# theAdamColton/dct-autoencoder

Measured on AMD Instinct MI355X. Metric: Mpix/s encode (DCT+PatchNorm+LFQ), patch14 512²; 1/2/4/8 GPU, %HBM roofline, higher is better.
Workload: dtype f32; 1 GPU; fused encode of 512x512 RGB images, patch14, max_patch 32x32, S=3072, LFQ 14 codebooks x 2^14, beta=0; global_batch=1024, parallelism=dp1 (image shards, no collective)

## Files before the change

dct-autoencoder_amd/csrc/dctae_fft2.hip:

```cpp
#include "dctae_device.h"
#include "dctae_fft_common.h"
#include "dctae_launch.h"
#include "dctae_spec512.h"

namespace dctae {

__device__ __forceinline__ constexpr int pad16(int m) { return m + (m >> 4); }

template <int N>
struct RowsLds {
  static constexpr int M = N / 2;
  static constexpr int MP = pad16(M - 1) + 2;
  float2 z[4][3][MP];
};

template <int N, int R1, int R2, typename Px>
__device__ __forceinline__ void rows2_item(const ImgDesc& d, int y_first, const Px* __restrict__ rgb,
                                           float* __restrict__ T, RowsLds<N>& L, const float2* post_s,
                                           const float2* tw_s, const ColorMats& cm) {
  constexpr int M = N / 2;
  constexpr int MP = RowsLds<N>::MP;
  constexpr int B1 = M / R1, B2 = M / R2;
  constexpr int PX = (N + 63) / 64;
  constexpr int KI = (M + 63) / 64;
// ... 458 lines not shown
        if (jl < KS && sk.codes) sk.codes[tok * KS + jl] = (uint16_t)code;
        if (sk.raw && jl < KS) {
#pragma unroll
          for (int p2 = 0; p2 < KS; ++p2) sk.raw[tok * KS * KS + jl * KS + p2] = row[p2];
        }
      }
    }
  } else {
    for (int h = g16; h < d.qh; h += 16) {
      float vals[KS];
      const float* row = zs + (KS * h + jl) * KSP;
#pragma unroll
      for (int p2 = 0; p2 < KS; ++p2) vals[p2] = row[p2];
      const int f = (h * d.qw + strip) * ep.C + c;
      token_epilogue_p<KS>(ep, c, h, strip, jl, vals, d.tok_off + f, sk);
    }
  }
}

template <bool THR, int IPB, bool PF>
__device__ __forceinline__ void cols7_block(int b, const ImgDesc* __restrict__ imgs, const int* __restrict__ list,
                                            int n_list, int n_items, int qw, const float* __restrict__ ws,
                                            const float2* __restrict__ tw, const float2* __restrict__ post,
                                            const EncParams& ep, const TokenSinks& sk, Cols7Lds& L, float4* post4,
                                            float2* tw_s, float* sbias) {
  constexpr int M = 256;
  const int per_x = (n_items + 7) / 8;
  const int slot = b >> 3;
  const int t = (b & 7) * per_x + slot % per_x, g = slot / per_x;
  const int k0 = g * IPB;
  if (t >= n_items || k0 >= n_list) return;
  const int c = t / qw, strip = t - c * qw;
  const float4* p4 = reinterpret_cast<const float4*>(post);
  for (int i = threadIdx.x; i < M + 1; i += 256) post4[i] = p4[i];
  for (int i = threadIdx.x; i < M; i += 256) tw_s[i] = tw[i];
  float2 thr_r[2][7];
  cols_thresholds<THR>(imgs[list[k0]], c, strip, ep, thr_r, sbias);
  float va[16], vb[16];
  {
    const ImgDesc d0 = imgs[list[k0]];
    cols7_load(d0, c, strip, ws + d0.ws_t, va, vb);
  }
  __syncthreads();
#pragma unroll
  for (int u = 0; u < IPB; ++u) {
    const int k = k0 + u;
    if (k < n_list) {
      const ImgDesc dk = imgs[list[k]];
      if (u > 0 && !PF) cols7_load(dk, c, strip, ws + dk.ws_t, va, vb);
#pragma unroll
      for (int r = 0; r < 16; ++r) asm volatile("" : "+v"(va[r]), "+v"(vb[r]));
      float na[16], nb[16];
      if (PF && u + 1 < IPB) {
        const ImgDesc dn = imgs[list[min(k + 1, n_list - 1)]];
        cols7_load(dn, c, strip, ws + dn.ws_t, na, nb);
      }
      cols7_compute<THR>(dk, c, strip, L, va, vb, post4, tw_s, sbias, thr_r, ep, sk);
      __syncthreads();
      if (PF && u + 1 < IPB) {
#pragma unroll
        for (int r = 0; r < 16; ++r) {
          va[r] = na[r];
          vb[r] = nb[r];
        }
      }
    }
  }
}

template <bool THR, int IPB, bool PF>
__global__ __launch_bounds__(256) void k_fft_cols7(const ImgDesc* __restrict__ imgs, const int* __restrict__ list,
                                                   int n_list, int n_items, int qw,
                                                   const float* __restrict__ ws, const float2* __restrict__ tw,
                                                   const float2* __restrict__ post, EncParams ep, TokenSinks sk) {
  __shared__ Cols7Lds L;
  __shared__ float4 post4[257];
  __shared__ float2 tw_s[256];
  __shared__ float sbias[32];
  cols7_block<THR, IPB, PF>(blockIdx.x, imgs, list, n_list, n_items, qw, ws, tw, post, ep, sk, L, post4, tw_s, sbias);
}

constexpr int kC5bIpb = 3;
constexpr int kC5bNormIpb = 3;
template <bool THR, int IPB, bool NORM = false>
__global__ __launch_bounds__(256) void k_cols512b(const ImgDesc* __restrict__ imgs, const int* __restrict__ list,
                                                  int n_list, const float* __restrict__ ws,
                                                  const float2* __restrict__ tw, const float2* __restrict__ post,
                                                  EncParams ep, TokenSinks sk) {
  constexpr int M = 256, per_x = 12;
  __shared__ Cols512bLds L;
  const int b = blockIdx.x;
  const int slot = b >> 3;
  const int t = (b & 7) * per_x + slot % per_x, k0 = (slot / per_x) * IPB;
  if (k0 >= n_list) return;
  const int c = t >> 5, strip = t & 31;
  const int tid = threadIdx.x;
  L.tw2[tid >> 4][tid & 15] = tw[(tid >> 4) * (tid & 15)];
  const float4* p4 = reinterpret_cast<const float4*>(post);
  {
    const float4 ab = p4[tid];
    L.pc[tid] = make_float4(ab.x + ab.z, ab.x - ab.z, ab.y + ab.w, ab.y - ab.w);
  }
  const float4 abM = p4[M];
  const float4 pcM = make_float4(abM.x + abM.z, abM.x - abM.z, abM.y + abM.w, abM.y - abM.w);
  float2 thr_r[2][7];
  cols_thresholds<THR>(imgs[list[k0]], c, strip, ep, thr_r, nullptr);
  float sb[2] = {0.0f, 0.0f};
  if (THR || NORM) {
    const int g16 = tid >> 4;
    sb[0] = __fdiv_rn(-(float)(g16 + strip), ep.ci[c]);
    sb[1] = __fdiv_rn(-(float)(g16 + 16 + strip), ep.ci[c]);
  }
  float2 tn[NORM ? 2 : 1][14];
  if constexpr (NORM) cols_norm_tables(c, strip, ep, tn);
  float4 qa[8];
  cols512b_load(c, strip, ws + imgs[list[k0]].ws_t, qa);
  __syncthreads();
#pragma unroll
  for (int u = 0; u < IPB; ++u) {
    const int k = k0 + u;
    if (k < n_list) {
      const ImgDesc dk = imgs[list[k]];
      t_opaque(qa);
      float4 qn[8];
      if (u + 1 < IPB) cols512b_load(c, strip, ws + imgs[list[min(k + 1, n_list - 1)]].ws_t, qn);
      float4 qf[8];
      t_decode(qa, qf);
      cols512b_compute<THR, NORM>(dk, c, strip, L, qf, pcM, sb, thr_r, ep, sk, tn);
      __syncthreads();
      if (u + 1 < IPB) {
#pragma unroll
        for (int r = 0; r < 8; ++r) qa[r] = qn[r];
      }
    }
  }
}

struct Cols512wLds {
  union {
    cf xch[28][kXchStridePk];
    float X[2][449 * 14];
  } u;
  uint32_t rmax[2][32][14];
  float2 tw2[16][16];
  float4 pc[256];
};

__device__ __forceinline__ void cols512w_load(int c, int kx, const float* __restrict__ T, float4 (&q)[8]) {
  t_load_column(c, kx, opaque_tid() & 15, T, q);
}

__device__ __forceinline__ void cols512w_transform(Cols512wLds& L, const float4 (&qa)[8], float4 pcM) {
#pragma clang fp contract(fast)
  constexpr int N = 512, M = 256, KS = 14;
  const int tid = opaque_tid();
  const int G = tid >> 4, j = tid & 15;
  const int sg = G >= KS ? 1 : 0, col = G - KS * sg;
  const int s = sigma16(j);
  const bool self0 = (j == 0), self8 = (j == 15);
  cf v[16];
#pragma unroll
  for (int bb = 0; bb < 8; ++bb) {
    v[bb] = (cf){qa[bb].x, qa[bb].y};
    v[15 - bb] = (cf){mirror16(qa[bb].z), mirror16(qa[bb].w)};
  }
  fft256_group(v, L.u.xch[G], j, s, L.tw2);
  __syncthreads();
  float* xs = L.u.X[sg];
  float* xa = xs + s * KS + col;
  float* xb = xs + (N - s) * KS + col;
  float4 cn0 = L.pc[s], cn1 = L.pc[s + 16];
#pragma unroll
  for (int i = 0; i < 16; i += 2) {
    const float4 c0 = cn0, c1 = cn1;
    if (i + 2 < 16) {
      cn0 = L.pc[s + 16 * (i + 2)];
      cn1 = L.pc[s + 16 * (i + 3)];
    }
    cf x0, x1;
    makhoul_step2(v, i, self0, self8, c0, c1, x0, x1);
    xa[224 * i] = x0.x;
    xa[224 * (i + 1)] = x1.x;
    if (i >= 4) xb[-224 * i] = x0.y;
    if (i + 1 >= 4) xb[-224 * (i + 1)] = x1.y;
  }
  if (self0) xs[M * KS + col] = (pcM.x + pcM.y) * v[0].x + (pcM.w - pcM.z) * v[0].y;
}

__device__ __forceinline__ void cols512w_epilogue(Cols512wLds& L, const ImgDesc& dk, int c, int sp,
                                                  const float2 (&thr_r)[2][7], const EncParams& ep,
                                                  const TokenSinks& sk) {
  constexpr int KS = 14;
  const int tid = opaque_tid();
  const int eh = tid / KS, ejl = tid - KS * eh;
  const f2v* row0 = reinterpret_cast<const f2v*>(L.u.X[0]) + (KS * eh + ejl) * (KS / 2);
  const f2v* row1 = reinterpret_cast<const f2v*>(L.u.X[1]) + (KS * eh + ejl) * (KS / 2);
  uint32_t code0 = 0, code1 = 0;
  float am0 = 0.0f, am1 = 0.0f;
#pragma unroll
  for (int p = 0; p < KS / 2; ++p) code_bits4(code0, code1, am0, am1, row0[p], row1[p], thr_r[0][p], thr_r[1][p]);
  L.rmax[0][eh][ejl] = __float_as_uint(am0);
  L.rmax[1][eh][ejl] = __float_as_uint(am1);
  if (sk.codes) {
    sk.codes[cols_tok(dk, c, 2 * sp, eh, ep.C) * KS + ejl] = (uint16_t)code0;
    sk.codes[cols_tok(dk, c, 2 * sp + 1, eh, ep.C) * KS + ejl] = (uint16_t)code1;
  }
  if (sk.raw) {
    for (int e = tid; e < 2 * 32 * 49; e += 448) {
      const int r = e / (32 * 49), e2 = e - r * 32 * 49, h = e2 / 49, q = e2 - h * 49;
      reinterpret_cast<float4*>(sk.raw + cols_tok(dk, c, 2 * sp + r, h, ep.C) * (KS * KS))[q] =
          reinterpret_cast<const float4*>(L.u.X[r] + KS * KS * h)[q];
// ... 10 lines not shown
    uint32_t m = 0;
#pragma unroll
    for (int q = 0; q < KS; ++q) m = max(m, L.rmax[r][h][q]);
    const float sb = __fdiv_rn(-(float)(h + 2 * sp + r), ep.ci[c]);
    sk.scores[cols_tok(dk, c, 2 * sp + r, h, ep.C)] = __fadd_rn(__fmul_rn(__uint_as_float(m), ep.mw), sb);
  }
}

template <int IPB>
__global__ __launch_bounds__(448) __attribute__((amdgpu_waves_per_eu(4))) void k_cols512w(
    const ImgDesc* __restrict__ imgs, const int* __restrict__ list, int n_list, const float* __restrict__ ws,
    const float2* __restrict__ tw, const float2* __restrict__ post, EncParams ep, TokenSinks sk) {
  constexpr int M = 256, KS = 14, per_x = 6;
  __shared__ Cols512wLds L;
  const int b = blockIdx.x;
  const int slot = b >> 3;
  const int t = (b & 7) * per_x + slot % per_x, k0 = (slot / per_x) * IPB;
  if (k0 >= n_list) return;
  const int c = t >> 4, sp = t & 15;
  {
    const int tid = threadIdx.x;
    if (tid < 256) {
      L.tw2[tid >> 4][tid & 15] = tw[(tid >> 4) * (tid & 15)];
      const float4 ab = reinterpret_cast<const float4*>(post)[tid];
      L.pc[tid] = make_float4(ab.x + ab.z, ab.x - ab.z, ab.y + ab.w, ab.y - ab.w);
    }
  }
  const float4 abM = reinterpret_cast<const float4*>(post)[M];
  const float4 pcM = make_float4(abM.x + abM.z, abM.x - abM.z, abM.y + abM.w, abM.y - abM.w);
  float2 thr_r[2][7];
  {
    const int tid = opaque_tid();
    const int eh = tid / KS, ejl = tid - KS * eh;
#pragma unroll
    for (int r = 0; r < 2; ++r) {
      const float2* t2 = reinterpret_cast<const float2*>(
          ep.thr + ((((int64_t)c * ep.maxph + eh) * ep.maxpw) + 2 * sp + r) * (KS * KS) + (int64_t)ejl * KS);
#pragma unroll
      for (int p = 0; p < KS / 2; ++p) thr_r[r][p] = t2[p];
    }
  }
  const int kx = [&] {
    const int G = opaque_tid() >> 4, sg = G >= KS ? 1 : 0;
    return KS * (2 * sp + sg) + G - KS * sg;
  }();
  float4 qa[8];
  cols512w_load(c, kx, ws + imgs[list[k0]].ws_t, qa);
  __syncthreads();
#pragma unroll
  for (int u = 0; u < IPB; ++u) {
    const int k = k0 + u;
    if (k >= n_list) break;
    t_opaque(qa);
    float4 qn[8];
    if (u + 1 < IPB) cols512w_load(c, kx, ws + imgs[list[min(k + 1, n_list - 1)]].ws_t, qn);
    if (u > 0) cols512w_scores(L, imgs[list[k - 1]], c, sp, ep, sk);
    float4 qf[8];
    t_decode(qa, qf);
    cols512w_transform(L, qf, pcM);
    __syncthreads();
    cols512w_epilogue(L, imgs[list[k]], c, sp, thr_r, ep, sk);
    __syncthreads();
    if (u + 1 < IPB) {
#pragma unroll
      for (int r = 0; r < 8; ++r) qa[r] = qn[r];
    }
  }
  cols512w_scores(L, imgs[list[min(k0 + IPB, n_list) - 1]], c, sp, ep, sk);
}

void launch_cols512b(const ImgDesc* imgs, const int* list, int n_list, const float* ws, const float2* tw,
                     const float2* post, const EncParams& ep, const TokenSinks& sk, hipStream_t s, bool wide) {
  if (n_list <= 0) return;
  const bool thr = ep.median && ep.thr && !sk.norm && ep.maxph <= 32 && ep.cb_dim == 14 && ep.ncb == 14;
  const bool norm = !thr && sk.norm && ep.median && !sk.raw && ep.maxph == 32 && ep.maxpw == 32 &&
                    (!sk.codes || (ep.cb_dim == 14 && ep.ncb == 14));
  const int ipb = thr ? kC5bIpb : norm ? kC5bNormIpb : 2;
  const int grid = 96 * ((n_list + ipb - 1) / ipb);
  if (thr && wide) {
    hipLaunchKernelGGL((k_cols512w<kC5bIpb>), dim3(48 * ((n_list + kC5bIpb - 1) / kC5bIpb)), dim3(448), 0, s, imgs,
                       list, n_list, ws, tw, post, ep, sk);
    return;
  }
  if (thr)
    hipLaunchKernelGGL((k_cols512b<true, kC5bIpb>), dim3(grid), dim3(256), 0, s, imgs, list, n_list, ws, tw, post, ep,
                       sk);
  else if (norm)
    hipLaunchKernelGGL((k_cols512b<false, kC5bNormIpb, true>), dim3(grid), dim3(256), 0, s, imgs, list, n_list, ws, tw,
                       post, ep, sk);
  else
    hipLaunchKernelGGL((k_cols512b<false, 2>), dim3(grid), dim3(256), 0, s, imgs, list, n_list, ws, tw, post, ep, sk);
}

int cols7_grid(int n_list, int qw, int ipb) {
  const int n_items = 3 * qw, per_x = (n_items + 7) / 8;
  return 8 * per_x * ((n_list + ipb - 1) / ipb);
}

template <int N, int R2, int KS, bool THR>
__global__ __launch_bounds__(256) void k_fft_cols4(const ImgDesc* __restrict__ imgs, const int4* __restrict__ blocks,
                                                   const float* __restrict__ ws, const float2* __restrict__ tw,
                                                   const float2* __restrict__ post, EncParams ep, TokenSinks sk) {
  constexpr int M = N / 2;
  __shared__ ColsLds<N> L;
  __shared__ float2 post_s[2 * (M + 1)];
  __shared__ float2 tw_s[M];
  __shared__ float sbias[32];
  for (int i = threadIdx.x; i < 2 * (M + 1); i += 256) post_s[i] = post[i];
  for (int i = threadIdx.x; i < M; i += 256) tw_s[i] = tw[i];
  const int4 jb = blocks[blockIdx.x];
  const ImgDesc d = imgs[jb.x];
  cols4_item<N, R2, KS, THR>(d, jb.y, jb.z, ws + d.ws_t, L.z, post_s, tw_s, sbias, ep, sk);
}

template <bool THR>
__global__ __launch_bounds__(256) void k_cols224(const ImgDesc* __restrict__ imgs, const int4* __restrict__ blocks,
                                                 int n_items, const float* __restrict__ ws,
                                                 const float2* __restrict__ tw, const float2* __restrict__ post,
                                                 EncParams ep, TokenSinks sk) {
#pragma clang fp contract(fast)
  constexpr int N = 224, M = 112, R1 = 16, R2 = 7, B1 = 7, KS = 14;
  constexpr int KSP = 30;
  static_assert(KSP >= 2 * KS, "28 columns");
  constexpr int ZROWS = 2 * (pad16(M - 1) + 1);
  static_assert(N <= ZROWS, "natural rows fit the complex layout");
  __shared__ float zs[ZROWS * KSP];
  __shared__ float4 pc[M + 1];
  __shared__ float2 tw_s[M];
  __shared__ float sbias[2][16];
  {
    const float4* p4 = reinterpret_cast<const float4*>(post);
    for (int i = threadIdx.x; i < M + 1; i += 256) {
      const float4 ab = p4[i];
      pc[i] = make_float4(ab.x + ab.z, ab.x - ab.z, ab.y + ab.w, ab.y - ab.w);
    }
    for (int i = threadIdx.x; i < M; i += 256) tw_s[i] = tw[i];
  }
  const int n_pairs = (n_items + 1) / 2, per_x = (n_pairs + 7) / 8;
  const int pidx = (int)(blockIdx.x & 7) * per_x + (int)(blockIdx.x >> 3);
  if (pidx >= n_pairs) return;
  const int tid = opaque_tid();
  const int i0 = 2 * pidx;
  const int4 ja = blocks[i0], jb = blocks[i0 + 1 < n_items ? i0 + 1 : i0];
  const ImgDesc da = imgs[ja.x], db = imgs[jb.x];
  const int g16 = tid >> 4, jl = tid & 15, jlc = min(jl, KS - 1);
  if (THR) {
    if (tid < 32) {
      const int u = tid >> 4, h = tid & 15;
      const int c = u ? jb.y : ja.y, strip = u ? jb.z : ja.z;
      sbias[u][h] = __fdiv_rn(-(float)(h + strip), ep.ci[c]);
    }
  }
  if (tid < 224) {
    const int u = tid >= 112 ? 1 : 0, t = tid - 112 * u;
    const int y0 = t / (KS / 2), p = t - y0 * (KS / 2);
    const int c = u ? jb.y : ja.y, strip = u ? jb.z : ja.z;
    const int64_t tbase = u ? db.ws_t : da.ws_t;
    const int H = u ? db.H : da.H, Kw = u ? db.Kw : da.Kw;
    const c4f2* src = reinterpret_cast<const c4f2*>(ws + tbase + ((int64_t)c * H + y0) * Kw + strip * KS) + p;
    const int64_t rstep = (int64_t)8 * Kw;
    c4f2 tv[N / 16];
#pragma unroll
    for (int k = 0; k < N / 16; ++k) tv[k] = src[k * rstep];
    float* dst = zs + y0 * KSP + KS * u + 2 * p;
#pragma unroll
    for (int k = 0; k < N / 16; ++k) {
      dst[16 * KSP * k] = tv[k].x;
// ... 238 lines not shown
```

dct-autoencoder_amd/csrc/dctae_rows512.h:

```cpp
#pragma once
#include "dctae_device.h"
#include "dctae_fft_common.h"
#include "dctae_pixel.h"

namespace dctae {

typedef unsigned v4u __attribute__((ext_vector_type(4)));

#ifndef DCTAE_TLAYOUT
#define DCTAE_TLAYOUT 2
#endif
static_assert(DCTAE_TLAYOUT == 0 || DCTAE_TLAYOUT == 2, "T' layouts: 0 or 2");
__device__ __forceinline__ int t4_index(int band4, int kx) {
#if DCTAE_TLAYOUT == 0
  return band4 * 448 + kx;
#else
  return ((band4 >> 2) * 448 + kx) * 4 + (band4 & 3);
#endif
}
constexpr int kTStAux = 2, kTLdAux = 2;

__device__ __forceinline__ int u4_index(int band4, int kx) { return ((band4 >> 2) * 448 + kx) * 4 + (band4 & 3); }
constexpr int kUStAux = 2;

// ... 34 lines not shown
  asm("v_pk_mul_f32 %0, %1, %2 op_sel_hi:[1,0] neg_hi:[1,0]" : "=v"(t) : "v"(A), "v"(c12));
  asm("v_pk_fma_f32 %0, %1, %2, %3 op_sel:[0,1,0] op_sel_hi:[1,1,1]" : "=v"(t) : "v"(P), "v"(c12), "v"(t));
  asm("v_pk_fma_f32 %0, %1, %2, %3 op_sel:[1,0,0] op_sel_hi:[0,0,1] neg_lo:[1,0,0] neg_hi:[1,0,0]"
      : "=v"(t) : "v"(A), "v"(c34), "v"(t));
  asm("v_pk_fma_f32 %0, %1, %2, %3 op_sel:[1,1,0] op_sel_hi:[0,1,1] neg_hi:[1,0,0]"
      : "=v"(t) : "v"(P), "v"(c34), "v"(t));
  return t;
}

__device__ __forceinline__ int sigma16(int j) { return j < 8 ? j : (j < 15 ? j + 1 : 8); }

__device__ __forceinline__ void fft256_group(cf (&v)[16], cf* xr, int j, int s, const float2 (&tw2)[16][16]) {
#pragma clang fp contract(fast)
  DFTV<16>::run(v);
#pragma unroll
  for (int k1 = 0; k1 < 16; ++k1) xr[16 * k1 + (j ^ (k1 & 14))] = v[k1];
  __builtin_amdgcn_fence(__ATOMIC_RELEASE, "wavefront");
  __builtin_amdgcn_wave_barrier();
  __builtin_amdgcn_fence(__ATOMIC_ACQUIRE, "wavefront");
  {
    const float4* rr = reinterpret_cast<const float4*>(xr + 16 * s);
    const int sw = s >> 1;
#pragma unroll
    for (int q = 0; q < 8; ++q) {
      const float4 a = rr[q ^ sw];
      v[2 * q] = (cf){a.x, a.y};
      v[2 * q + 1] = (cf){a.z, a.w};
    }
  }
  __builtin_amdgcn_fence(__ATOMIC_RELEASE, "wavefront");
  __builtin_amdgcn_wave_barrier();
#pragma unroll
  for (int r = 1; r < 16; ++r) {
    const float2 w = tw2[r][s];
    v[r] = cmul_pk(v[r], (cf){w.x, w.y});
  }
  DFTV<16>::run(v);
}

__device__ __forceinline__ cf makhoul_step(const cf (&v)[16], int i, int s, bool self0, bool self8,
                                           const float4* pc) {
  const cf m = (cf){mirror16(v[15 - i].x), mirror16(v[15 - i].y)};
  const cf own = self0 ? v[(16 - i) & 15] : v[15 - i];
  const cf P = (self0 || self8) ? own : m;
  const float4 cc = pc[s + 16 * i];
  return makhoul_pair(v[i], P, (cf){cc.x, cc.y}, (cf){cc.z, cc.w});
}

__device__ __forceinline__ void makhoul_pair2(cf A0, cf P0, float4 c0, cf A1, cf P1, float4 c1, cf& t0, cf& t1) {
  const cf c12a = (cf){c0.x, c0.y}, c34a = (cf){c0.z, c0.w}, c12b = (cf){c1.x, c1.y}, c34b = (cf){c1.z, c1.w};
  asm("v_pk_mul_f32 %0, %2, %3 op_sel_hi:[1,0] neg_hi:[1,0]\n\t"
      "v_pk_mul_f32 %1, %6, %7 op_sel_hi:[1,0] neg_hi:[1,0]\n\t"
      "v_pk_fma_f32 %0, %4, %3, %0 op_sel:[0,1,0] op_sel_hi:[1,1,1]\n\t"
      "v_pk_fma_f32 %1, %8, %7, %1 op_sel:[0,1,0] op_sel_hi:[1,1,1]\n\t"
      "v_pk_fma_f32 %0, %2, %5, %0 op_sel:[1,0,0] op_sel_hi:[0,0,1] neg_lo:[1,0,0] neg_hi:[1,0,0]\n\t"
      "v_pk_fma_f32 %1, %6, %9, %1 op_sel:[1,0,0] op_sel_hi:[0,0,1] neg_lo:[1,0,0] neg_hi:[1,0,0]\n\t"
      "v_pk_fma_f32 %0, %4, %5, %0 op_sel:[1,1,0] op_sel_hi:[0,1,1] neg_hi:[1,0,0]\n\t"
      "v_pk_fma_f32 %1, %8, %9, %1 op_sel:[1,1,0] op_sel_hi:[0,1,1] neg_hi:[1,0,0]"
      : "=&v"(t0), "=&v"(t1)
      : "v"(A0), "v"(c12a), "v"(P0), "v"(c34a), "v"(A1), "v"(c12b), "v"(P1), "v"(c34b));
}

__device__ __forceinline__ void makhoul_step2(const cf (&v)[16], int i, bool self0, bool self8, float4 c0, float4 c1,
                                              cf& x0, cf& x1) {
  (void)self0;
  (void)self8;
  float p0x, p0y, p1x, p1y, q0x, q0y, q1x, q1y;
  asm("s_mov_b32 vcc_lo, 0x00010001\n\t"
      "s_mov_b32 vcc_hi, 0x00010001\n\t"
      "v_cndmask_b32 %4, %8, %12, vcc\n\t"
      "v_cndmask_b32 %5, %9, %13, vcc\n\t"
      "v_cndmask_b32 %6, %10, %8, vcc\n\t"
      "v_cndmask_b32 %7, %11, %9, vcc\n\t"
      "s_mov_b32 vcc_lo, 0x80018001\n\t"
      "s_mov_b32 vcc_hi, 0x80018001\n\t"
      "v_cndmask_b32_dpp %0, %8, %4, vcc row_mirror row_mask:0xf bank_mask:0xf\n\t"
      "v_cndmask_b32_dpp %1, %9, %5, vcc row_mirror row_mask:0xf bank_mask:0xf\n\t"
      "v_cndmask_b32_dpp %2, %10, %6, vcc row_mirror row_mask:0xf bank_mask:0xf\n\t"
      "v_cndmask_b32_dpp %3, %11, %7, vcc row_mirror row_mask:0xf bank_mask:0xf"
      : "=&v"(p0x), "=&v"(p0y), "=&v"(p1x), "=&v"(p1y), "=&v"(q0x), "=&v"(q0y), "=&v"(q1x), "=&v"(q1y)
      : "v"(v[15 - i].x), "v"(v[15 - i].y), "v"(v[14 - i].x), "v"(v[14 - i].y), "v"(v[(16 - i) & 15].x),
        "v"(v[(16 - i) & 15].y)
      : "vcc");
  makhoul_pair2(v[i], (cf){p0x, p0y}, c0, v[i + 1], (cf){p1x, p1y}, c1, x0, x1);
}

__device__ __forceinline__ void xpose4_rows(float (&r)[4]) {
  const auto a = __builtin_amdgcn_permlane32_swap(__float_as_uint(r[0]), __float_as_uint(r[2]), false, false);
  const auto b = __builtin_amdgcn_permlane32_swap(__float_as_uint(r[1]), __float_as_uint(r[3]), false, false);
  const auto c = __builtin_amdgcn_permlane16_swap(a[0], b[0], false, false);
  const auto d = __builtin_amdgcn_permlane16_swap(a[1], b[1], false, false);
  r[0] = __uint_as_float(c[0]);
  r[1] = __uint_as_float(c[1]);
  r[2] = __uint_as_float(d[0]);
  r[3] = __uint_as_float(d[1]);
}

template <bool band, typename Px>
__device__ __forceinline__ void rows512_item_pk(Rows512XchPk& X, const Rows512Tab& L, const Px* __restrict__ img,
                                                int H, int y0, float* T, uint32_t plane_bytes, const ColorMats& cm) {
#pragma clang fp contract(fast)
  constexpr int N = 512, M = 256, KW = 448;
  const int tid = threadIdx.x;
  const int wv = tid >> 6, g = (tid >> 4) & 3, j = tid & 15;
  const int y = y0 + 4 * wv + g;
  const int yl = min(y, H - 1);
  const int64_t hw = (int64_t)H * N;
  const Px* src = img + (int64_t)yl * N + 4 * j;

  float4 I[3][8];
  if constexpr (sizeof(Px) == 4) {
#pragma unroll
    for (int b = 0; b < 8; ++b) {
      I[0][b] = *reinterpret_cast<const float4*>(src + 64 * b);
      I[1][b] = *reinterpret_cast<const float4*>(src + hw + 64 * b);
      I[2][b] = *reinterpret_cast<const float4*>(src + 2 * hw + 64 * b);
    }
  } else {
    uint32_t U[3][8];
#pragma unroll
    for (int b = 0; b < 8; ++b) {
      U[0][b] = *reinterpret_cast<const uint32_t*>(src + 64 * b);
      U[1][b] = *reinterpret_cast<const uint32_t*>(src + hw + 64 * b);
      U[2][b] = *reinterpret_cast<const uint32_t*>(src + 2 * hw + 64 * b);
    }
#pragma unroll
    for (int b = 0; b < 8; ++b)
#pragma unroll
      for (int c = 0; c < 3; ++c)
        I[c][b] = make_float4(unit_from_dword(U[c][b], 0), unit_from_dword(U[c][b], 1), unit_from_dword(U[c][b], 2),
                              unit_from_dword(U[c][b], 3));
  }
  cf A[3][8], B[3][8];
#pragma unroll
  for (int b = 0; b < 8; ++b) {
    const cf r01 = (cf){I[0][b].x, I[0][b].y}, r23 = (cf){I[0][b].z, I[0][b].w};
    const cf g01 = (cf){I[1][b].x, I[1][b].y}, g23 = (cf){I[1][b].z, I[1][b].w};
    const cf b01 = (cf){I[2][b].x, I[2][b].y}, b23 = (cf){I[2][b].z, I[2][b].w};
    cf p02[3], p31[3];
#pragma unroll
    for (int i = 0; i < 3; ++i) {
      const cf l01 = splat_mix(cm.rgb2lms, i, r01, g01, b01);
      const cf l23 = splat_mix(cm.rgb2lms, i, r23, g23, b23);
      const cf lg01 = (cf){__builtin_amdgcn_logf(fabsf(l01.x)), __builtin_amdgcn_logf(fabsf(l01.y))};
      const cf lg23 = (cf){__builtin_amdgcn_logf(fabsf(l23.x)), __builtin_amdgcn_logf(fabsf(l23.y))};
      const cf k = (cf){0.430000007152557373046875f, 0.430000007152557373046875f};
      const cf e01 = k * lg01, e23 = k * lg23;
      p02[i] = (cf){__builtin_copysignf(__builtin_amdgcn_exp2f(e01.x), l01.x),
                    __builtin_copysignf(__builtin_amdgcn_exp2f(e23.x), l23.x)};
      p31[i] = (cf){__builtin_copysignf(__builtin_amdgcn_exp2f(e23.y), l23.y),
                    __builtin_copysignf(__builtin_amdgcn_exp2f(e01.y), l01.y)};
    }
#pragma unroll
    for (int c = 0; c < 3; ++c) {
      A[c][b] = splat_mix(cm.lms2ipt, c, p02[0], p02[1], p02[2]);
      B[c][b] = splat_mix(cm.lms2ipt, c, p31[0], p31[1], p31[2]);
    }
  }

  cf* xr = X.xch[wv][g];
  const int s = sigma16(j);
  const bool self0 = (j == 0), self8 = (j == 15);
  const int rowo = (y * KW + s) * 4;
  const int rown = (y * KW + (N - 15 * 16) - s) * 4;
  const int rown4 = s >= 1 ? rown : 0x7ffffff0;

// ... 106 lines not shown
```

dct-autoencoder_amd/csrc/dctae_spec512.h:

```cpp
#pragma once
#include "dctae_device.h"
#include "dctae_fft_common.h"
#include "dctae_rows512.h"

namespace dctae {

__device__ __forceinline__ int opaque_tid() {
  int t;
  asm volatile("v_mov_b32 %0, %1" : "=v"(t) : "v"((int)threadIdx.x));
  return t;
}

typedef float f2v __attribute__((ext_vector_type(2)));

template <bool THR>
__device__ __forceinline__ void cols_thresholds(const ImgDesc& d, int c, int strip, const EncParams& ep,
                                                 float2 (&thr_r)[2][7], float* sbias) {
  constexpr int KS = 14, EPR = 2;
  const int tid = opaque_tid();
  const int g16 = tid >> 4, jl = tid & 15;
#if defined(DCTAE_PROFILING) && defined(DCTAE_C7_ABL)
  if (DCTAE_C7_ABL & 4) {
#pragma unroll
    for (int r = 0; r < EPR; ++r)
// ... 45 lines not shown
  float* Xf = reinterpret_cast<float*>(const_cast<f2v*>(X2));
  auto store_tokens = [&](float* dst) { cols_store_tokens(d, c, strip, Xf, dst, ep.C); };
  if (THR) {
#pragma unroll
    for (int r = 0; r < EPR; ++r) {
      const int h = g16 + 16 * r;
      if (h < d.qh) {
        const f2v* row = X2 + (KS * h + (jl < KS ? jl : 0)) * (KS / 2);
        uint32_t am = 0, code = 0;
#pragma unroll
        for (int p = 0; p < KS / 2; ++p) {
          const f2v v2 = row[p];
          am = max(am, max(__float_as_uint(v2.x) & 0x7fffffffu, __float_as_uint(v2.y) & 0x7fffffffu));
          code = 2 * code + (v2.x >= thr_r[r][p].x ? 1u : 0u);
          code = 2 * code + (v2.y >= thr_r[r][p].y ? 1u : 0u);
        }
        am = jl < KS ? am : 0u;
        am = max(am, (uint32_t)__builtin_amdgcn_mov_dpp((int)am, 0x128, 0xf, 0xf, false));
        am = max(am, (uint32_t)__builtin_amdgcn_mov_dpp((int)am, 0x124, 0xf, 0xf, false));
        am = max(am, (uint32_t)__builtin_amdgcn_mov_dpp((int)am, 0x122, 0xf, 0xf, false));
        am = max(am, (uint32_t)__builtin_amdgcn_mov_dpp((int)am, 0x121, 0xf, 0xf, false));
        const int64_t tok = tok_of(h);
        if (jl == 0) sk.scores[tok] = __fadd_rn(__fmul_rn(__uint_as_float(am), ep.mw), sb[r]);
        if (jl < KS && sk.codes) sk.codes[tok * KS + jl] = (uint16_t)code;
      }
    }
    if (sk.raw) store_tokens(sk.raw);
  } else {
    const bool norm = sk.norm && ep.median;
    if (sk.raw) {
      store_tokens(sk.raw);
      if (norm) __syncthreads();
    }
    TokenSinks sc = sk;
    sc.raw = nullptr;
    sc.norm = nullptr;
    for (int h = g16; h < d.qh; h += 16) {
      float vals[KS];
      f2v* row = reinterpret_cast<f2v*>(Xf) + (KS * h + (jl < KS ? jl : 0)) * (KS / 2);
#pragma unroll
      for (int p = 0; p < KS / 2; ++p) {
        const f2v v2 = row[p];
        vals[2 * p] = v2.x;
        vals[2 * p + 1] = v2.y;
      }
      const int64_t tok = tok_of(h);
      if (norm) {
        float y[KS];
        token_epilogue_p<KS>(ep, c, h, strip, jl, vals, tok, sc, y);
        if (jl < KS) {
#pragma unroll
          for (int p = 0; p < KS / 2; ++p) row[p] = (f2v){y[2 * p], y[2 * p + 1]};
        }
      } else {
        token_epilogue_p<KS>(ep, c, h, strip, jl, vals, tok, sc);
      }
    }
    if (norm) {
      __syncthreads();
      store_tokens(sk.norm);
    }
  }
}

__device__ __forceinline__ void code_bits4(uint32_t& c0, uint32_t& c1, float& a0, float& a1, f2v x, f2v y,
                                           float2 tx, float2 ty) {
  uint64_t m0, m1, m2, m3;
  asm("v_cmp_ge_f32_e64 %[m0], %[x0], %[t0]\n\t"
      "v_cmp_ge_f32_e64 %[m1], %[x1], %[t1]\n\t"
      "v_cmp_ge_f32_e64 %[m2], %[y0], %[u0]\n\t"
      "v_cmp_ge_f32_e64 %[m3], %[y1], %[u1]\n\t"
      "v_maximum3_f32 %[a0], |%[x0]|, |%[x1]|, %[a0]\n\t"
      "v_maximum3_f32 %[a1], |%[y0]|, |%[y1]|, %[a1]\n\t"
      "v_addc_co_u32_e64 %[c0], %[m0], %[c0], %[c0], %[m0]\n\t"
      "v_addc_co_u32_e64 %[c0], %[m1], %[c0], %[c0], %[m1]\n\t"
      "v_addc_co_u32_e64 %[c1], %[m2], %[c1], %[c1], %[m2]\n\t"
      "v_addc_co_u32_e64 %[c1], %[m3], %[c1], %[c1], %[m3]"
      : [c0] "+v"(c0), [c1] "+v"(c1), [a0] "+v"(a0), [a1] "+v"(a1), [m0] "=&s"(m0), [m1] "=&s"(m1),
        [m2] "=&s"(m2), [m3] "=&s"(m3)
      : [x0] "v"(x.x), [x1] "v"(x.y), [y0] "v"(y.x), [y1] "v"(y.y), [t0] "v"(tx.x), [t1] "v"(tx.y),
        [u0] "v"(ty.x), [u1] "v"(ty.y));
}

__device__ __forceinline__ void cols512b_epilogue(const ImgDesc& d, int c, int strip, const f2v* X2,
                                                  const float (&sb)[2], const float2 (&thr_r)[2][7],
                                                  const EncParams& ep, const TokenSinks& sk) {
  constexpr int KS = 14;
  const int tid = opaque_tid();
  const int g16 = tid >> 4, jl = min(tid & 15, KS - 1);
  const bool im = (d.tband & 2) != 0;
  const int64_t tok0 = d.tok_off + (im ? (int64_t)(c * d.qw + strip) * d.qh : (int64_t)strip * ep.C + c);
  const uint32_t hs = im ? 1u : (uint32_t)(d.qw * ep.C);
  const f2v* row0 = X2 + (KS * g16 + jl) * (KS / 2);
  const f2v* row1 = row0 + 16 * KS * (KS / 2);
  uint32_t code0 = 0, code1 = 0;
  float am0 = 0.0f, am1 = 0.0f;
#pragma unroll
  for (int p = 0; p < KS / 2; ++p) code_bits4(code0, code1, am0, am1, row0[p], row1[p], thr_r[0][p], thr_r[1][p]);
  uint32_t u0 = __float_as_uint(am0), u1 = __float_as_uint(am1);
#define DCTAE_ROR_MAX(ctl)                                                        \
  u0 = max(u0, (uint32_t)__builtin_amdgcn_mov_dpp((int)u0, ctl, 0xf, 0xf, false)); \
  u1 = max(u1, (uint32_t)__builtin_amdgcn_mov_dpp((int)u1, ctl, 0xf, 0xf, false));
  DCTAE_ROR_MAX(0x128) DCTAE_ROR_MAX(0x124) DCTAE_ROR_MAX(0x122) DCTAE_ROR_MAX(0x121)
#undef DCTAE_ROR_MAX
  const uint32_t span = 31 * hs + 1;
  const uint32_t o0 = (uint32_t)g16 * hs, o1 = o0 + 16 * hs;
  const auto srs = __builtin_amdgcn_make_buffer_rsrc(sk.scores + tok0, 0, (int)(span * 4), 0x00020000);
  __builtin_amdgcn_raw_buffer_store_b32(__float_as_uint(__fadd_rn(__fmul_rn(__uint_as_float(u0), ep.mw), sb[0])),
                                        srs, o0 * 4, 0, 0);
  __builtin_amdgcn_raw_buffer_store_b32(__float_as_uint(__fadd_rn(__fmul_rn(__uint_as_float(u1), ep.mw), sb[1])),
                                        srs, o1 * 4, 0, 0);
  if (sk.codes) {
    const auto crs = __builtin_amdgcn_make_buffer_rsrc(sk.codes + tok0 * KS, 0, (int)(span * KS * 2), 0x00020000);
    __builtin_amdgcn_raw_buffer_store_b16((uint16_t)code0, crs, (o0 * KS + jl) * 2, 0, 0);
    __builtin_amdgcn_raw_buffer_store_b16((uint16_t)code1, crs, (o1 * KS + jl) * 2, 0, 0);
  }
  if (sk.raw) cols_store_tokens(d, c, strip, reinterpret_cast<const float*>(X2), sk.raw, ep.C);
}

__device__ __forceinline__ constexpr int z7addr(int m) { return 16 * (m ^ ((m >> 3) & 1)); }

__device__ __forceinline__ int cols7_j2(int w, int g) {
  const int a = (g & 2) ? 2 * w + 1 : 2 * w;
  const int base = (w == 0 && g < 2) ? (g ? 8 : 0) : ((g & 1) ? (g & 2 ? 15 - 2 * w : 16 - 2 * w) : a);
  return base;
}

__device__ __forceinline__ void cols7_load(const ImgDesc& d, int c, int strip, const float* __restrict__ T,
                                           float (&va)[16], float (&vb)[16]) {
  constexpr int N = 512;
  const int tid = opaque_tid();
  const int j1 = tid >> 4, col = min(tid & 15, 13);
  const int rs = d.Kw;
  const float* cb = T + (int64_t)c * N * rs + strip * 14;
  const auto rsrc = __builtin_amdgcn_make_buffer_rsrc(const_cast<float*>(cb), 0, N * rs * 4, 0x00020000);
  const int lo = (4 * j1 * rs + col) * 4;
  const int hi = ((2 * N - 1 - 4 * j1 - 64 * 15) * rs + col) * 4;
  const int step = 64 * rs * 4, two = 2 * rs * 4;
  constexpr int aux = 0;
#pragma unroll
  for (int r = 0; r < 8; ++r) {
    va[r] = __uint_as_float(__builtin_amdgcn_raw_buffer_load_b32(rsrc, lo, r * step, aux));
    vb[r] = __uint_as_float(__builtin_amdgcn_raw_buffer_load_b32(rsrc, lo + two, r * step, aux));
  }
#pragma unroll
  for (int r = 8; r < 16; ++r) {
    va[r] = __uint_as_float(__builtin_amdgcn_raw_buffer_load_b32(rsrc, hi, (15 - r) * step, aux));
    vb[r] = __uint_as_float(__builtin_amdgcn_raw_buffer_load_b32(rsrc, hi - two, (15 - r) * step, aux));
  }
}

__device__ __forceinline__ float partner_row(float x, bool even_row) {
  const auto r = __builtin_amdgcn_permlane16_swap(__float_as_uint(x), __float_as_uint(x), false, false);
  return __uint_as_float(even_row ? r[1] : r[0]);
}

union Cols7Lds {
  float2 z[256 * 16];
  float X[449 * 14];
};

template <bool W0>
__device__ __forceinline__ void cols7_post(const cf (&v)[16], int j2, int g, int col, const float4* post4,
                                           float* Xs) {
#pragma clang fp contract(fast)
  constexpr int N = 512, M = 256, KS = 14;
  const int colc = col < KS ? col : KS - 1;
  const bool self = W0 && g < 2;
  float* xa = Xs + j2 * KS + colc;
  float* xb = Xs + (N - j2 - 16 * 15) * KS + colc;
  const float4* ps = post4 + j2;
#pragma unroll
  for (int i = 0; i < 16; ++i) {
    cf P;
    P.x = __int_as_float(__builtin_amdgcn_ds_swizzle(__float_as_int(v[15 - i].x), 0x401f));
    P.y = __int_as_float(__builtin_amdgcn_ds_swizzle(__float_as_int(v[15 - i].y), 0x401f));
    if (W0) P = self ? ((j2 == 0) ? v[(16 - i) & 15] : v[15 - i]) : P;
    const cf A = v[i];
    const float4 ab = ps[16 * i];
    const cf al = (cf){ab.x, ab.y}, be = (cf){ab.z, ab.w};
    const cf s1 = add_conj(A, P), d1 = sub_conj(A, P);
    const cf W = fma_iw(d1, be, fma_x(d1, be, fma_iw(s1, al, mul_x(s1, al))));
    xa[224 * i] = W.x;
    if (i >= 4) xb[224 * (15 - i)] = -W.y;
  }
  if (W0 && j2 == 0) {
    const cf A = v[0];
    const float4 ab = post4[M];
    const cf s1 = add_conj(A, A), d1 = sub_conj(A, A);
    const cf W = fma_iw(d1, (cf){ab.z, ab.w}, fma_x(d1, (cf){ab.z, ab.w}, cmul_pk(s1, (cf){ab.x, ab.y})));
    Xs[M * KS + colc] = W.x;
  }
}

template <bool THR>
__device__ __forceinline__ void cols7_compute(const ImgDesc& d, int c, int strip, Cols7Lds& L, const float (&va)[16],
                                              const float (&vb)[16], const float4* post4, const float2* tw_s,
                                              const float* sbias, const float2 (&thr_r)[2][7], const EncParams& ep,
                                              const TokenSinks& sk) {
#pragma clang fp contract(fast)
// ... 79 lines not shown

__device__ __forceinline__ void cols512b_load(int c, int strip, const float* __restrict__ T, float4 (&q)[8]) {
  const int tid = opaque_tid();
  const int G = tid >> 4, j = tid & 15;
  constexpr int KW = 448;
  const auto rsrc = __builtin_amdgcn_make_buffer_rsrc(const_cast<float*>(T) + (int64_t)c * 512 * KW, 0, 512 * KW * 4,
                                                      0x00020000);
  const int kx = 14 * strip + min(G, 13);
  const int o = t4_index(j, kx) * 16;
  constexpr int bstep = 16 * KW * 16;
#if defined(DCTAE_PROFILING) && defined(DCTAE_C5B_ABL)
  if (DCTAE_C5B_ABL & 4) {
#pragma unroll
    for (int b = 0; b < 8; ++b) q[b] = make_float4(0.001f * (b + j), 0.002f * kx, 0.003f * c, 0.0004f * b);
    return;
  }
#endif
#pragma unroll
  for (int b = 0; b < 8; ++b)
    q[b] = __builtin_bit_cast(float4, __builtin_amdgcn_raw_buffer_load_b128(rsrc, o, b * bstep, kTLdAux));
}

__device__ __forceinline__ void cols512b_norm_epilogue(const ImgDesc& d, int c, int strip, float* Xf,
                                                       const float (&sb)[2], const float2 (&tn)[2][14],
                                                       const EncParams& ep, const TokenSinks& sk) {
  constexpr int KS = 14;
  const int tid = opaque_tid();
  const int g16 = tid >> 4, jl = tid & 15, jlc = min(jl, KS - 1);
#pragma unroll
  for (int r = 0; r < 2; ++r) {
    const int h = g16 + 16 * r;
    f2v* row = reinterpret_cast<f2v*>(Xf) + (KS * h + jlc) * (KS / 2);
    float y[KS];
    uint32_t am = 0, code = 0;
#pragma unroll
    for (int p = 0; p < KS / 2; ++p) {
      const f2v v2 = row[p];
      am = max(am, max(__float_as_uint(v2.x) & 0x7fffffffu, __float_as_uint(v2.y) & 0x7fffffffu));
#pragma unroll
      for (int e = 0; e < 2; ++e) {
        const float x = e ? v2.y : v2.x;
        const float2 t = tn[r][2 * p + e];
        const float q = __fdiv_rn(__fsub_rn(x, t.x), t.y);
        const float v = (q != q) ? q : fminf(fmaxf(q, ep.min_val), ep.max_val);
        y[2 * p + e] = v;
        code = 2 * code + (v > 0.0f ? 1u : 0u);
      }
    }
    am = jl < KS ? am : 0u;
    am = max(am, (uint32_t)__builtin_amdgcn_mov_dpp((int)am, 0x128, 0xf, 0xf, false));
    am = max(am, (uint32_t)__builtin_amdgcn_mov_dpp((int)am, 0x124, 0xf, 0xf, false));
    am = max(am, (uint32_t)__builtin_amdgcn_mov_dpp((int)am, 0x122, 0xf, 0xf, false));
    am = max(am, (uint32_t)__builtin_amdgcn_mov_dpp((int)am, 0x121, 0xf, 0xf, false));
    const int64_t tok = cols_tok(d, c, strip, h, ep.C);
    if (jl == 0) sk.scores[tok] = __fadd_rn(__fmul_rn(__uint_as_float(am), ep.mw), sb[r]);
    if (jl < KS) {
      if (sk.codes) sk.codes[tok * KS + jl] = (uint16_t)code;
#pragma unroll
      for (int p = 0; p < KS / 2; ++p) row[p] = (f2v){y[2 * p], y[2 * p + 1]};
    }
  }
  __syncthreads();
  cols_store_tokens(d, c, strip, Xf, sk.norm, ep.C);
}

__device__ __forceinline__ void cols_norm_tables(int c, int strip, const EncParams& ep, float2 (&tn)[2][14]) {
  constexpr int KS = 14;
  const int tid = opaque_tid();
  const int g16 = tid >> 4, jlc = min(tid & 15, KS - 1);
#pragma unroll
  for (int r = 0; r < 2; ++r) {
    const int64_t tab = ((((int64_t)c * ep.maxph + g16 + 16 * r) * ep.maxpw) + strip) * (KS * KS) + (int64_t)jlc * KS;
    const float2* m2 = reinterpret_cast<const float2*>(ep.median + tab);
    const float2* b2 = reinterpret_cast<const float2*>(ep.b + tab);
#pragma unroll
    for (int p = 0; p < KS / 2; ++p) {
      const float2 mv = m2[p], bv = b2[p];
      tn[r][2 * p] = make_float2(mv.x, __fadd_rn(__fmul_rn(bv.x, 1.41421353816986083984375f), ep.eps));
      tn[r][2 * p + 1] = make_float2(mv.y, __fadd_rn(__fmul_rn(bv.y, 1.41421353816986083984375f), ep.eps));
    }
  }
}

template <bool THR, bool NORM = false>
__device__ __forceinline__ void cols512b_compute(const ImgDesc& d, int c, int strip, Cols512bLds& L,
                                                 const float4 (&q)[8], const float4 pcM, const float (&sb)[2],
                                                 const float2 (&thr_r)[2][7], const EncParams& ep,
                                                 const TokenSinks& sk, const float2 (*tn)[14] = nullptr) {
#pragma clang fp contract(fast)
  constexpr int N = 512, M = 256, KS = 14;
  const int tid = opaque_tid();
  const int G = tid >> 4, j = tid & 15;
  const int colc = min(G, KS - 1);
  const int s = sigma16(j);
  const bool self0 = (j == 0), self8 = (j == 15);
  cf v[16];
#pragma unroll
  for (int b = 0; b < 8; ++b) {
    v[b] = (cf){q[b].x, q[b].y};
    v[15 - b] = (cf){mirror16(q[b].z), mirror16(q[b].w)};
  }
  fft256_group(v, L.u.xch[G], j, s, L.tw2);
  __syncthreads();
#if defined(DCTAE_PROFILING) && defined(DCTAE_C5B_ABL)
  if (DCTAE_C5B_ABL & 2) {
    cf acc = v[0];
#pragma unroll
    for (int i = 1; i < 16; ++i) acc += v[i];
    L.u.X[tid] = acc.x + acc.y;
    __syncthreads();
    return;
  }
#endif
  float* xa = L.u.X + s * KS + colc;
  float* xb = L.u.X + (N - s) * KS + colc;
  float4 cn0 = L.pc[s], cn1 = L.pc[s + 16];
#pragma unroll
  for (int i = 0; i < 16; i += 2) {
    const float4 c0 = cn0, c1 = cn1;
    if (i + 2 < 16) {
      cn0 = L.pc[s + 16 * (i + 2)];
      cn1 = L.pc[s + 16 * (i + 3)];
    }
    cf x0, x1;
    makhoul_step2(v, i, self0, self8, c0, c1, x0, x1);
    xa[224 * i] = x0.x;
    xa[224 * (i + 1)] = x1.x;
    if (i >= 4) xb[-224 * i] = x0.y;
    if (i + 1 >= 4) xb[-224 * (i + 1)] = x1.y;
  }
  if (self0) L.u.X[M * KS + colc] = (pcM.x + pcM.y) * v[0].x + (pcM.w - pcM.z) * v[0].y;
  __syncthreads();
#if defined(DCTAE_PROFILING) && defined(DCTAE_C5B_ABL)
  if (DCTAE_C5B_ABL & 1) return;
#endif
  if (THR)
    cols512b_epilogue(d, c, strip, reinterpret_cast<const f2v*>(L.u.X), sb, thr_r, ep, sk);
  else if (NORM)
    cols512b_norm_epilogue(d, c, strip, L.u.X, sb, *reinterpret_cast<const float2(*)[2][14]>(tn), ep, sk);
  else
    cols_epilogue<false>(d, c, strip, reinterpret_cast<const f2v*>(L.u.X), sb, thr_r, ep, sk);
}

}
```

Before: 156,500 Mpix/s.

## Use wave-private LDS regions for Makhoul post in codes-only cols512b path

Adds a PRIV variant of the 512-column kernel, used when thresholded codes are needed without raw tokens. Each group writes its Makhoul post-processing output into its own region of the exchange buffer, so one barrier and the shared X staging layout are dropped. The epilogue then reads its transposed coefficients from those private regions. The Makhoul step also takes its lane masks from SGPRs instead of rebuilding vcc each time. This risks LDS bank conflicts in the strided epilogue reads and depends on the private regions fitting inside the exchange buffer.

```diff
diff --git a/dct-autoencoder_amd/csrc/dctae_fft2.hip b/dct-autoencoder_amd/csrc/dctae_fft2.hip
--- a/dct-autoencoder_amd/csrc/dctae_fft2.hip
+++ b/dct-autoencoder_amd/csrc/dctae_fft2.hip
@@ -564,7 +564,7 @@
 
 constexpr int kC5bIpb = 3;
 constexpr int kC5bNormIpb = 3;
-template <bool THR, int IPB, bool NORM = false>
+template <bool THR, int IPB, bool NORM = false, bool PRIV = false>
 __global__ __launch_bounds__(256) void k_cols512b(const ImgDesc* __restrict__ imgs, const int* __restrict__ list,
                                                   int n_list, const float* __restrict__ ws,
                                                   const float2* __restrict__ tw, const float2* __restrict__ post,
@@ -608,7 +608,7 @@
       if (u + 1 < IPB) cols512b_load(c, strip, ws + imgs[list[min(k + 1, n_list - 1)]].ws_t, qn);
       float4 qf[8];
       t_decode(qa, qf);
-      cols512b_compute<THR, NORM>(dk, c, strip, L, qf, pcM, sb, thr_r, ep, sk, tn);
+      cols512b_compute<THR, NORM, PRIV>(dk, c, strip, L, qf, pcM, sb, thr_r, ep, sk, tn);
       __syncthreads();
       if (u + 1 < IPB) {
 #pragma unroll
@@ -785,7 +785,10 @@
                        list, n_list, ws, tw, post, ep, sk);
     return;
   }
-  if (thr)
+  if (thr && !sk.raw)
+    hipLaunchKernelGGL((k_cols512b<true, kC5bIpb, false, true>), dim3(grid), dim3(256), 0, s, imgs, list, n_list, ws, tw,
+                       post, ep, sk);
+  else if (thr)
     hipLaunchKernelGGL((k_cols512b<true, kC5bIpb>), dim3(grid), dim3(256), 0, s, imgs, list, n_list, ws, tw, post, ep,
                        sk);
   else if (norm)
diff --git a/dct-autoencoder_amd/csrc/dctae_rows512.h b/dct-autoencoder_amd/csrc/dctae_rows512.h
--- a/dct-autoencoder_amd/csrc/dctae_rows512.h
+++ b/dct-autoencoder_amd/csrc/dctae_rows512.h
@@ -140,6 +140,33 @@
       : "v"(v[15 - i].x), "v"(v[15 - i].y), "v"(v[14 - i].x), "v"(v[14 - i].y), "v"(v[(16 - i) & 15].x),
         "v"(v[(16 - i) & 15].y)
       : "vcc");
+  makhoul_pair2(v[i], (cf){p0x, p0y}, c0, v[i + 1], (cf){p1x, p1y}, c1, x0, x1);
+}
+
+struct MakhoulMasks {
+  uint64_t self0, ends;
+  __device__ __forceinline__ static MakhoulMasks get() {
+    MakhoulMasks m = {0x0001000100010001ull, 0x8001800180018001ull};
+    asm volatile("" : "+s"(m.self0), "+s"(m.ends));
+    return m;
+  }
+};
+
+__device__ __forceinline__ void makhoul_step2(const cf (&v)[16], int i, const MakhoulMasks& mk, float4 c0, float4 c1,
+                                              cf& x0, cf& x1) {
+  float p0x, p0y, p1x, p1y, q0x, q0y, q1x, q1y;
+  register uint64_t ends asm("vcc") = mk.ends;
+  asm("v_cndmask_b32_e64 %4, %8, %12, %14\n\t"
+      "v_cndmask_b32_e64 %5, %9, %13, %14\n\t"
+      "v_cndmask_b32_e64 %6, %10, %8, %14\n\t"
+      "v_cndmask_b32_e64 %7, %11, %9, %14\n\t"
+      "v_cndmask_b32_dpp %0, %8, %4, vcc row_mirror row_mask:0xf bank_mask:0xf\n\t"
+      "v_cndmask_b32_dpp %1, %9, %5, vcc row_mirror row_mask:0xf bank_mask:0xf\n\t"
+      "v_cndmask_b32_dpp %2, %10, %6, vcc row_mirror row_mask:0xf bank_mask:0xf\n\t"
+      "v_cndmask_b32_dpp %3, %11, %7, vcc row_mirror row_mask:0xf bank_mask:0xf"
+      : "=&v"(p0x), "=&v"(p0y), "=&v"(p1x), "=&v"(p1y), "=&v"(q0x), "=&v"(q0y), "=&v"(q1x), "=&v"(q1y)
+      : "v"(v[15 - i].x), "v"(v[15 - i].y), "v"(v[14 - i].x), "v"(v[14 - i].y), "v"(v[(16 - i) & 15].x),
+        "v"(v[(16 - i) & 15].y), "s"(mk.self0), "s"(ends));
   makhoul_pair2(v[i], (cf){p0x, p0y}, c0, v[i + 1], (cf){p1x, p1y}, c1, x0, x1);
 }
 
diff --git a/dct-autoencoder_amd/csrc/dctae_spec512.h b/dct-autoencoder_amd/csrc/dctae_spec512.h
--- a/dct-autoencoder_amd/csrc/dctae_spec512.h
+++ b/dct-autoencoder_amd/csrc/dctae_spec512.h
@@ -151,6 +151,10 @@
         [u0] "v"(ty.x), [u1] "v"(ty.y));
 }
 
+constexpr int kPrivRegion = 2 * kXchStridePk;
+__device__ __forceinline__ constexpr int cols512b_priv_off(int G) { return kPrivRegion * G + 16 * (G & 1); }
+
+template <bool PRIV = false>
 __device__ __forceinline__ void cols512b_epilogue(const ImgDesc& d, int c, int strip, const f2v* X2,
                                                   const float (&sb)[2], const float2 (&thr_r)[2][7],
                                                   const EncParams& ep, const TokenSinks& sk) {
@@ -160,12 +164,22 @@
   const bool im = (d.tband & 2) != 0;
   const int64_t tok0 = d.tok_off + (im ? (int64_t)(c * d.qw + strip) * d.qh : (int64_t)strip * ep.C + c);
   const uint32_t hs = im ? 1u : (uint32_t)(d.qw * ep.C);
-  const f2v* row0 = X2 + (KS * g16 + jl) * (KS / 2);
-  const f2v* row1 = row0 + 16 * KS * (KS / 2);
   uint32_t code0 = 0, code1 = 0;
   float am0 = 0.0f, am1 = 0.0f;
-#pragma unroll
-  for (int p = 0; p < KS / 2; ++p) code_bits4(code0, code1, am0, am1, row0[p], row1[p], thr_r[0][p], thr_r[1][p]);
+  if constexpr (PRIV) {
+    const float* x0 = reinterpret_cast<const float*>(X2) + KS * g16 + jl;
+    const float* x1 = x0 + 16 * KS;
+#pragma unroll
+    for (int p = 0; p < KS / 2; ++p) {
+      const int oa = cols512b_priv_off(2 * p), ob = cols512b_priv_off(2 * p + 1);
+      code_bits4(code0, code1, am0, am1, (f2v){x0[oa], x0[ob]}, (f2v){x1[oa], x1[ob]}, thr_r[0][p], thr_r[1][p]);
+    }
+  } else {
+    const f2v* row0 = X2 + (KS * g16 + jl) * (KS / 2);
+    const f2v* row1 = row0 + 16 * KS * (KS / 2);
+#pragma unroll
+    for (int p = 0; p < KS / 2; ++p) code_bits4(code0, code1, am0, am1, row0[p], row1[p], thr_r[0][p], thr_r[1][p]);
+  }
   uint32_t u0 = __float_as_uint(am0), u1 = __float_as_uint(am1);
 #define DCTAE_ROR_MAX(ctl)                                                        \
   u0 = max(u0, (uint32_t)__builtin_amdgcn_mov_dpp((int)u0, ctl, 0xf, 0xf, false)); \
@@ -184,7 +198,8 @@
     __builtin_amdgcn_raw_buffer_store_b16((uint16_t)code0, crs, (o0 * KS + jl) * 2, 0, 0);
     __builtin_amdgcn_raw_buffer_store_b16((uint16_t)code1, crs, (o1 * KS + jl) * 2, 0, 0);
   }
-  if (sk.raw) cols_store_tokens(d, c, strip, reinterpret_cast<const float*>(X2), sk.raw, ep.C);
+  if constexpr (!PRIV)
+    if (sk.raw) cols_store_tokens(d, c, strip, reinterpret_cast<const float*>(X2), sk.raw, ep.C);
 }
 
 __device__ __forceinline__ constexpr int z7addr(int m) { return 16 * (m ^ ((m >> 3) & 1)); }
@@ -430,12 +445,13 @@
   }
 }
 
-template <bool THR, bool NORM = false>
+template <bool THR, bool NORM = false, bool PRIV = false>
 __device__ __forceinline__ void cols512b_compute(const ImgDesc& d, int c, int strip, Cols512bLds& L,
                                                  const float4 (&q)[8], const float4 pcM, const float (&sb)[2],
                                                  const float2 (&thr_r)[2][7], const EncParams& ep,
                                                  const TokenSinks& sk, const float2 (*tn)[14] = nullptr) {
 #pragma clang fp contract(fast)
+  static_assert(!PRIV || (THR && !NORM), "the wave-private post serves the codes-only epilogue");
   constexpr int N = 512, M = 256, KS = 14;
   const int tid = opaque_tid();
   const int G = tid >> 4, j = tid & 15;
@@ -449,6 +465,31 @@
     v[15 - b] = (cf){mirror16(q[b].z), mirror16(q[b].w)};
   }
   fft256_group(v, L.u.xch[G], j, s, L.tw2);
+  if constexpr (PRIV) {
+    float* xg = reinterpret_cast<float*>(&L.u.xch[0][0]) + cols512b_priv_off(G);
+    float* xa = xg + s;
+    float* xb = xg + (N - s);
+    const MakhoulMasks mk = MakhoulMasks::get();
+    float4 cn0 = L.pc[s], cn1 = L.pc[s + 16];
+#pragma unroll
+    for (int i = 0; i < 16; i += 2) {
+      const float4 c0 = cn0, c1 = cn1;
+      if (i + 2 < 16) {
+        cn0 = L.pc[s + 16 * (i + 2)];
+        cn1 = L.pc[s + 16 * (i + 3)];
+      }
+      cf x0, x1;
+      makhoul_step2(v, i, mk, c0, c1, x0, x1);
+      xa[16 * i] = x0.x;
+      xa[16 * (i + 1)] = x1.x;
+      if (i >= 4) xb[-16 * i] = x0.y;
+      if (i + 1 >= 4) xb[-16 * (i + 1)] = x1.y;
+    }
+    if (self0) xg[M] = (pcM.x + pcM.y) * v[0].x + (pcM.w - pcM.z) * v[0].y;
+    __syncthreads();
+    cols512b_epilogue<true>(d, c, strip, reinterpret_cast<const f2v*>(&L.u.xch[0][0]), sb, thr_r, ep, sk);
+    return;
+  }
   __syncthreads();
 #if defined(DCTAE_PROFILING) && defined(DCTAE_C5B_ABL)
   if (DCTAE_C5B_ABL & 2) {
```

New measurement: 157,000 Mpix/s (median of 2 runs). No clear change (+0.3%).
